# coreyjadams/SparseEventID

Hardware: NVIDIA B200
Metric: 3D sparse ResNet train events/sec (higher is better)
Workload: dtype bf16

## Files before the change

sparseeventid_b200/csrc/conv_tc.cu:

```cuda
#include <cstdlib>
#include <cstring>

#include "common.cuh"
#include "tc_ptx.cuh"

namespace tc {

constexpr int BM = 128;
constexpr int KC = 64;
constexpr int KC_TF32 = 32;
constexpr int A_BYTES = BM * 128;
constexpr int EPI_WARPS = 4;
constexpr int NGRP = 4;
constexpr int PROD_WARPS = 4 * NGRP;
constexpr int WARP_MMA = EPI_WARPS + PROD_WARPS;
constexpr int MMA_WARPS = 4;
constexpr int WARP_BLOAD = WARP_MMA + MMA_WARPS;
constexpr int THREADS = 32 * (WARP_BLOAD + 1);
constexpr int MAX_A = 12, MAX_B = 8;
constexpr int MASK_BYTES = 32;
constexpr int LIST_BYTES = 64 * 8;
using namespace tcptx;

__device__ __forceinline__ uint64_t make_desc_sw128(uint32_t saddr) {
  uint64_t d = 0;
  d |= (uint64_t)((saddr & 0x3FFFFu) >> 4);
  d |= (uint64_t)1 << 16;
  d |= (uint64_t)(1024 >> 4) << 32;
  d |= (uint64_t)1 << 46;
  d |= (uint64_t)2 << 61;
  return d;
}
__device__ __forceinline__ const unsigned char* mad_wide16(uint32_t units, const unsigned char* base) {
  uint64_t r;
  asm("mad.wide.u32 %0, %1, 16, %2;" : "=l"(r) : "r"(units), "l"((uint64_t)(uintptr_t)base));
  return reinterpret_cast<const unsigned char*>((uintptr_t)r);
}
template <bool TF32>
__device__ __forceinline__ uint32_t make_idesc(int n) {
  constexpr uint32_t fmt = TF32 ? 2u : 1u;
  return (1u << 4) | (fmt << 7) | (fmt << 10) | ((uint32_t)(n >> 3) << 17) | ((uint32_t)(BM >> 4) << 24);
}
template <bool TF32>
__device__ __forceinline__ void store8(void* out, int64_t idx, const float* f) {
  if constexpr (TF32) {
    float4* d = reinterpret_cast<float4*>(reinterpret_cast<float*>(out) + idx);
    d[0] = make_float4(f[0], f[1], f[2], f[3]);
    d[1] = make_float4(f[4], f[5], f[6], f[7]);
  } else {
    uint4 u;
    u.x = pack_bf16x2(f[0], f[1]); u.y = pack_bf16x2(f[2], f[3]);
    u.z = pack_bf16x2(f[4], f[5]); u.w = pack_bf16x2(f[6], f[7]);
    *reinterpret_cast<uint4*>(reinterpret_cast<__nv_bfloat16*>(out) + idx) = u;
  }
}
struct Params {
  const void* in;
  const int32_t* nbr;
  const unsigned char* bimg;
  const float* bias;
  void* out;
  int64_t n_rows, n_pad;
  int K, n_in, n_out;
  int nch;
  int last_kc;
  int T;
  int SA, SB;
  int num_tiles;
  int NM;
  int nbuf;
  int ksplit;
  unsigned long long* dbg;
  int exp;
};

template <int NCH, bool PAIR, bool TF32 = false>
__global__ void __launch_bounds__(THREADS, 1) k_conv_tc(const Params p) {
  static_assert(!(TF32 && PAIR), "a 32-channel fp32 row fills a stage");
  constexpr int ESZ = TF32 ? 4 : 2;
  constexpr int KCE = 128 / ESZ;
  const int nch = NCH > 0 ? NCH : p.nch;
  extern __shared__ unsigned char smem_raw[];
  pdl_launch_dependents();
  const uint32_t raw = smem_u32(smem_raw);
  const uint32_t base = (raw + 1023u) & ~1023u;
  unsigned char* gbase = smem_raw + (base - raw);
  const int SA = p.SA, SB = p.SB;
  const uint32_t b_bytes = (uint32_t)p.n_out * 128u;
  const uint32_t a_base = base;
  const uint32_t b_base = base + (uint32_t)SA * A_BYTES;
  const uint32_t bar0 = b_base + (uint32_t)SB * b_bytes;
  auto afull = [&](int s) { return bar0 + 8u * (uint32_t)s; };
  auto aempty = [&](int s) { return bar0 + 8u * (uint32_t)(MAX_A + s); };
  auto bfull = [&](int s) { return bar0 + 8u * (uint32_t)(2 * MAX_A + s); };
  auto bempty = [&](int s) { return bar0 + 8u * (uint32_t)(2 * MAX_A + MAX_B + s); };
  auto accf = [&](int b) { return bar0 + 8u * (uint32_t)(2 * MAX_A + 2 * MAX_B + b); };
  auto acce = [&](int b) { return bar0 + 8u * (uint32_t)(2 * MAX_A + 2 * MAX_B + 2 + b); };
  constexpr int NBAR = 2 * MAX_A + 2 * MAX_B + 4;
  unsigned char* tail = gbase + (size_t)SA * A_BYTES + (size_t)SB * b_bytes + 8 * NBAR;
  uint32_t* tmem_slot = reinterpret_cast<uint32_t*>(tail);
  uint32_t* amask = reinterpret_cast<uint32_t*>(tail + 16);
  unsigned char* lists = tail + 16 + MAX_A * MASK_BYTES;

  const int warp = __shfl_sync(0xffffffffu, (int)(threadIdx.x >> 5), 0), lane = threadIdx.x & 31;
  auto mark = [&](int role, int stage, int ev) {
#ifdef SCN_TC_TIMELINE
    if (p.dbg != nullptr && blockIdx.x == 0 && lane == 0 && stage < 256)
      p.dbg[((size_t)role * 256 + stage) * 8 + ev] = (unsigned long long)clock64();
#else
    (void)role; (void)stage; (void)ev;
#endif
  };
#ifdef SCN_TC_TIMELINE
  const int exp_flags = p.exp;
#else
  constexpr int exp_flags = 0;
#endif

  const int T = p.T;
  const int tile_lo = (int)(((int64_t)p.num_tiles * blockIdx.x) / gridDim.x);
  const int tile_hi = (int)(((int64_t)p.num_tiles * (blockIdx.x + 1)) / gridDim.x);
  const int my_tiles = tile_hi - tile_lo;
  const int my_groups = (my_tiles + T - 1) / T;
  auto tiles_in_group = [&](int g) { return my_tiles - g * T < T ? my_tiles - g * T : T; };
  const int NSTEP = PAIR ? (p.K + 1) / 2 : p.K;
  const int Q = NSTEP * nch;
  const bool ksplit = p.ksplit != 0 && p.NM == 2 && my_tiles == 1;

  if (warp == WARP_MMA) {
    if (lane == 0) {
      for (int s = 0; s < SA; ++s) {
        mbar_init(afull(s), 132);
        mbar_init(aempty(s), 1);
      }
      for (int s = 0; s < SB; ++s) {
        mbar_init(bfull(s), 1);
        mbar_init(bempty(s), ksplit ? 1 : p.NM);
      }
      for (int b = 0; b < 2; ++b) {
        mbar_init(accf(b), p.NM);
        mbar_init(acce(b), EPI_WARPS);
      }
      asm volatile("fence.mbarrier_init.release.cluster;" ::: "memory");
    }
    __syncwarp();
    asm volatile("tcgen05.alloc.cta_group::1.sync.aligned.shared::cta.b32 [%0], %1;" ::"r"(smem_u32(tmem_slot)), "r"(512)
                 : "memory");
    asm volatile("tcgen05.relinquish_alloc_permit.cta_group::1.sync.aligned;" ::: "memory");
  }
  tc_fence_before();
  __syncthreads();
  tc_fence_after();
  const uint32_t tmem_base = *tmem_slot;
  pdl_wait();

  const int NM = p.NM;
  const int spc = SA / NM;

  if (warp >= EPI_WARPS && warp < EPI_WARPS + PROD_WARPS) {
    const int pw = warp - EPI_WARPS;
    const int grp = pw >> 2, wq = pw & 3;
    const int cls = grp % NM, sub = grp / NM, gpc = NGRP / NM;
    constexpr int LPI = PAIR ? 4 : 8;
    constexpr int IPP = 32 / LPI;
    const int chunk = lane % LPI, isub = lane / LPI;
    const uint32_t row_vec = (uint32_t)p.n_in >> (TF32 ? 2 : 3);
    const int last_chunks = p.last_kc * ESZ / 16;
    const uint32_t lt = (1u << lane) - 1u;
    const uint32_t csw = (uint32_t)chunk << 4;
    const uint32_t myrow = 32u * (uint32_t)wq + (uint32_t)lane;
    const uint32_t drow = a_base + (myrow << 7) + ((myrow & 7u) << 4);

    int t = cls, q = 0, cc = 0, g = 0, tv = my_groups > 0 ? tiles_in_group(0) : 0;
    const int32_t* gptr = p.nbr + (int64_t)tile_lo * BM + myrow;
    const int32_t* qptr = gptr;
    const int64_t qstride = (int64_t)p.n_pad * (PAIR ? 2 : 1);
    auto next_q = [&]() {
      ++q;
      if (++cc == nch) { cc = 0; qptr += qstride; }
    };
    auto step = [&]() {
      if (ksplit) {
        next_q(); next_q();
        if (q >= Q) { g = my_groups; tv = 0; }
        return;
      }
      t += NM;
      if (t >= tv) {
        t = cls;
        next_q();
        if (q == Q) {
          q = 0; ++g;
          gptr += (int64_t)T * BM;
          qptr = gptr;
          tv = g < my_groups ? tiles_in_group(g) : 0;
        }
      }
    };
    auto valid = [&]() { return g < my_groups && (ksplit ? q < Q : cls < tv); };
    if (ksplit) {
      t = 0;
      if (cls == 1) next_q();
    }
    for (int i = 0; i < sub; ++i)
      if (valid()) step();
    auto fetch = [&](int& jl_, int& jh_, int& q_) {
      q_ = -1; jl_ = -1; jh_ = -1;
      if (valid()) {
        const int32_t* src = qptr + t * BM;
        jl_ = ldg_nc32(src);
        if (PAIR && (2 * q + 1 < p.K)) jh_ = ldg_nc32(src + p.n_pad);
        q_ = (q << 3) | cc;
        for (int i = 0; i < gpc; ++i) step();
      }
    };

    int ls = sub;
    uint32_t round = 0;
    int it = 0;
    auto do_stage = [&](const int jl, const int jh, const int qc) {
      if (wq == 0) mark(grp, it, 0);
      int2* list = reinterpret_cast<int2*>(lists + (pw * 2 + (it & 1)) * LIST_BYTES);
      const int slot = cls * spc + ls;
      const int ccur = qc & 7;
      const bool full = qc < (ksplit ? 16 : 8);
      const uint32_t dst = drow + (uint32_t)slot * A_BYTES;
      const uint32_t bl = __ballot_sync(0xffffffffu, jl >= 0);
      const uint32_t bh = PAIR ? __ballot_sync(0xffffffffu, jh >= 0) : 0u;
      int nlive;
      if (full) {
        list[lane] = make_int2(jl >= 0 ? (int)((uint32_t)jl * row_vec) : -1, (int)dst);
        if (PAIR) list[32 + lane] = make_int2(jh >= 0 ? (int)((uint32_t)jh * row_vec) : -1, (int)(dst ^ 0x40u));
        nlive = PAIR ? 64 : 32;
      } else {
        const int2 el = make_int2((int)((uint32_t)jl * row_vec), (int)dst);
        const int2 eh = make_int2((int)((uint32_t)jh * row_vec), (int)(dst ^ 0x40u));
        if (jl >= 0) list[__popc(bl & lt)] = el;
        nlive = __popc(bl);
        if (PAIR) {
          if (jh >= 0) list[nlive + __popc(bh & lt)] = eh;
          nlive += __popc(bh);
        }
        if (nlive & (IPP - 1)) {
          const bool from_hi = PAIR && bh != 0u;
          const int top = 31 - __clz(from_hi ? bh : bl);
          const int lx = __shfl_sync(0xffffffffu, from_hi ? eh.x : el.x, top);
          const int ly = __shfl_sync(0xffffffffu, from_hi ? eh.y : el.y, top);
          const int padded = (nlive + IPP - 1) & ~(IPP - 1);
          if (nlive + lane < padded) list[nlive + lane] = make_int2(lx, ly);
        }
      }
      __syncwarp();
      if (wq == 0) mark(grp, it, 1);

      mbar_wait(aempty(slot), (round & 1u) ^ 1u);
      if (wq == 0) mark(grp, it, 2);
      if (lane == 0) {
        amask[slot * 8 + wq] = ~bl;
        if (PAIR) amask[slot * 8 + 4 + wq] = ~bh;
      }
      const int npass = (nlive + IPP - 1) / IPP;
      const bool lane_on = PAIR ? true : chunk < (ccur == nch - 1 ? last_chunks : 8);
      const unsigned char* src0 = reinterpret_cast<const unsigned char*>(p.in) + ((uint32_t)ccur * 128u + csw);
      if (lane_on && !(exp_flags & 1)) {
        if (!full) {
          for (int p0 = 0; p0 < npass; p0 += 4) {
            int2 e[4];
#pragma unroll
            for (int u = 0; u < 4; ++u)
              if (p0 + u < npass) e[u] = list[(p0 + u) * IPP + isub];
#pragma unroll
            for (int u = 0; u < 4; ++u)
              if (p0 + u < npass) cp_async16((uint32_t)e[u].y ^ csw, mad_wide16((uint32_t)e[u].x, src0), 16u);
          }
        } else {
#pragma unroll
          for (int pass = 0; pass < 8; ++pass) {
            const int2 e = list[pass * IPP + isub];
            const bool live = e.x != -1;
            cp_async16((uint32_t)e.y ^ csw, mad_wide16(live ? (uint32_t)e.x : 0u, src0), live ? 16u : 0u);
          }
        }
      }
      cp_async_arrive_noinc(afull(slot));
      if (lane == 0) mbar_arrive(afull(slot));
      if (wq == 0) mark(grp, it, 3);
      ++it;
      ls += gpc;
      if (ls >= spc) { ls -= spc; ++round; }
    };

    int jlA, jhA, qA, jlB, jhB, qB;
    fetch(jlA, jhA, qA);
    fetch(jlB, jhB, qB);
    while (qA >= 0) {
      int jlC, jhC, qC;
      fetch(jlC, jhC, qC);
      do_stage(jlA, jhA, qA);
      jlA = jlB; jhA = jhB; qA = qB;
      jlB = jlC; jhB = jhC; qB = qC;
    }
  } else if (warp == WARP_BLOAD) {
    const int total_b = my_groups * Q;
    int bslot = 0;
    uint32_t bround = 0;
    for (int i = 0; i < total_b; ++i) {
      mark(8, i, 0);
      if (ksplit) mbar_wait_sleep(bempty(bslot), (bround & 1u) ^ 1u, 100u);
      else mbar_wait(bempty(bslot), (bround & 1u) ^ 1u);
      mark(8, i, 1);
      if (elect_one()) {
        mbar_expect_tx(bfull(bslot), b_bytes);
        bulk_g2s(b_base + (uint32_t)bslot * b_bytes, p.bimg + (size_t)(i % Q) * b_bytes, b_bytes, bfull(bslot));
      }
      __syncwarp();
      if (++bslot == SB) { bslot = 0; ++bround; }
    }
  } else if (warp >= WARP_MMA && warp < WARP_MMA + MMA_WARPS) {
    const int m = warp - WARP_MMA;
    if (m < NM) {
      const uint32_t idesc = make_idesc<TF32>(p.n_out);
      const uint64_t da0 = make_desc_sw128(a_base), db0 = make_desc_sw128(b_base);
      const int nbuf = p.nbuf;
      int bslot = 0;
      uint32_t bround = 0;
      int ls = 0;
      uint32_t around = 0;
      int it = 0;
      auto issue_stage = [&](int q, uint32_t col, uint64_t db, bool first) {
        const int cc = PAIR ? 0 : q % nch;
        const int step = PAIR ? q : q / nch;
        const int nk = PAIR ? ((2 * step + 1 < p.K) ? 4 : 2) : ((cc == nch - 1 ? p.last_kc : KCE) * ESZ / 32);
        const int aslot = m * spc + ls;
        mark(4 + m, it, 0);
        mbar_wait(afull(aslot), around & 1u);
        mark(4 + m, it, 1);
        tc_fence_after();
        uint32_t m0 = 0, m1 = 0, m2 = 0, m3 = 0, h0 = 0, h1 = 0, h2 = 0, h3 = 0;
        if (!first) {
          const uint4 mw = *reinterpret_cast<const uint4*>(amask + aslot * 8);
          m0 = __ballot_sync(0xffffffffu, (mw.x >> lane) & 1u);
          m1 = __ballot_sync(0xffffffffu, (mw.y >> lane) & 1u);
          m2 = __ballot_sync(0xffffffffu, (mw.z >> lane) & 1u);
          m3 = __ballot_sync(0xffffffffu, (mw.w >> lane) & 1u);
          if (PAIR) {
            const uint4 hw = *reinterpret_cast<const uint4*>(amask + aslot * 8 + 4);
            h0 = __ballot_sync(0xffffffffu, (hw.x >> lane) & 1u);
            h1 = __ballot_sync(0xffffffffu, (hw.y >> lane) & 1u);
            h2 = __ballot_sync(0xffffffffu, (hw.z >> lane) & 1u);
            h3 = __ballot_sync(0xffffffffu, (hw.w >> lane) & 1u);
          }
        }
        const uint64_t da = da0 + (uint64_t)((uint32_t)aslot * (A_BYTES >> 4));
        const uint32_t tmem_d = tmem_base + col;
        if (elect_one()) {
#pragma unroll
          for (int kk = 0; kk < 4; ++kk) {
            if (kk < nk && !(exp_flags & 2)) {
              const bool hi = PAIR && kk >= 2;
              umma_masked<TF32>(tmem_d, da + (uint64_t)(kk * 2), db + (uint64_t)(kk * 2), idesc, (!first || kk > 0) ? 1u : 0u,
                                hi ? h0 : m0, hi ? h1 : m1, hi ? h2 : m2, hi ? h3 : m3);
            }
          }
          umma_commit(aempty(aslot));
        }
        __syncwarp();
        mark(4 + m, it, 2);
        ++it;
        if (++ls == spc) { ls = 0; ++around; }
      };
      if (ksplit) {
        mbar_wait(acce(0), 1u);
        tc_fence_after();
        bslot = m;
        for (int q = m; q < Q; q += 2) {
          mbar_wait(bfull(bslot), bround & 1u);
          issue_stage(q, (uint32_t)(m * p.n_out), db0 + (uint64_t)(((uint32_t)bslot * b_bytes) >> 4), q < 2);
          if (elect_one()) umma_commit(bempty(bslot));
          __syncwarp();
          bslot += 2;
          if (bslot >= SB) { bslot -= SB; ++bround; }
        }
        if (elect_one()) umma_commit(accf(0));
        __syncwarp();
      } else
      for (int g = 0; g < my_groups; ++g) {
        const int buf = nbuf == 2 ? (g & 1) : 0;
        const uint32_t use = (uint32_t)(nbuf == 2 ? (g >> 1) : g);
        const int tv = tiles_in_group(g);
        mbar_wait(acce(buf), (use & 1u) ^ 1u);
        tc_fence_after();
        for (int q = 0; q < Q; ++q) {
          mark(10 + m, g * Q + q, 0);
          mbar_wait(bfull(bslot), bround & 1u);
          mark(10 + m, g * Q + q, 1);
          const uint64_t db = db0 + (uint64_t)(((uint32_t)bslot * b_bytes) >> 4);
          for (int t = m; t < tv; t += NM) issue_stage(q, (uint32_t)buf * 256u + (uint32_t)(t * p.n_out), db, q == 0);
          if (elect_one()) umma_commit(bempty(bslot));
          __syncwarp();
          if (++bslot == SB) { bslot = 0; ++bround; }
        }
        if (elect_one()) umma_commit(accf(buf));
        __syncwarp();
      }
    }
  } else if (warp < EPI_WARPS) {
    if (ksplit) {
      mbar_wait_sleep(accf(0), 0u, 100u);
      tc_fence_after();
      const int64_t row = (int64_t)tile_lo * BM + warp * 32 + lane;
      const uint32_t taddr = tmem_base + ((uint32_t)(warp * 32) << 16);
      for (int c0 = 0; c0 < p.n_out; c0 += 16) {
        uint32_t a[16], b[16];
        tmem_ld16x2(taddr + (uint32_t)c0, taddr + (uint32_t)(p.n_out + c0), a, b);
        if (row < p.n_rows && !(exp_flags & 4)) {
#pragma unroll
          for (int gq = 0; gq < 2; ++gq) {
            float f[8];
#pragma unroll
            for (int e = 0; e < 8; ++e)
              f[e] = __uint_as_float(a[gq * 8 + e]) + __uint_as_float(b[gq * 8 + e]) +
                     (p.bias ? __ldg(p.bias + c0 + gq * 8 + e) : 0.f);
            store8<TF32>(p.out, row * p.n_out + c0 + gq * 8, f);
          }
        }
      }
      tc_fence_before();
    } else
    for (int g = 0; g < my_groups; ++g) {
      const int buf = p.nbuf == 2 ? (g & 1) : 0;
      if (warp == 0) mark(9, g, 0);
      mbar_wait_long(accf(buf), (uint32_t)(p.nbuf == 2 ? (g >> 1) : g) & 1u);
      if (warp == 0) mark(9, g, 1);
      tc_fence_after();
      const int tv = tiles_in_group(g);
      for (int t = 0; t < tv; ++t) {
        const int64_t tile = (int64_t)tile_lo + (int64_t)g * T + t;
        const int64_t row = tile * BM + warp * 32 + lane;
        const uint32_t taddr = tmem_base + ((uint32_t)(warp * 32) << 16) + (uint32_t)buf * 256u + (uint32_t)(t * p.n_out);
        for (int c0 = 0; c0 < p.n_out; c0 += 32) {
          uint32_t v[32];
          tmem_ld32(taddr + (uint32_t)c0, v);
          if (row < p.n_rows && !(exp_flags & 4)) {
#pragma unroll
            for (int gq = 0; gq < 4; ++gq) {
              float f[8];
#pragma unroll
              for (int e = 0; e < 8; ++e)
                f[e] = __uint_as_float(v[gq * 8 + e]) + (p.bias ? __ldg(p.bias + c0 + gq * 8 + e) : 0.f);
              store8<TF32>(p.out, row * p.n_out + c0 + gq * 8, f);
            }
          }
        }
      }
      tc_fence_before();
      __syncwarp();
      if (warp == 0) mark(9, g, 2);
      if (lane == 0) mbar_arrive(acce(buf));
    }
  }

  tc_fence_before();
  __syncthreads();
  if (warp == WARP_MMA) {
    tc_fence_after();
    asm volatile("tcgen05.dealloc.cta_group::1.sync.aligned.b32 %0, %1;" ::"r"(tmem_base), "r"(512) : "memory");
  }
}

__global__ void k_prep_weights_tc(const float* __restrict__ W, int K, int Cin, int Cout, int transpose, int mirror,
                                  int nch, int pair, int tf32, void* __restrict__ img) {
  const int n_in = transpose ? Cout : Cin, n_out = transpose ? Cin : Cout;
  int64_t total = (int64_t)K * n_in * n_out;
  int64_t i = blockIdx.x * (int64_t)blockDim.x + threadIdx.x;
  if (i >= total) return;
  int k = (int)(i / ((int64_t)n_in * n_out));
  int rem = (int)(i - (int64_t)k * n_in * n_out);
  int n = rem / n_in, c = rem % n_in;
  int src_k = (transpose && mirror) ? K - 1 - k : k;
  int ci = transpose ? n : c, co = transpose ? c : n;
  float v = W[((int64_t)src_k * Cin + ci) * Cout + co];
  if (tf32) {
    const int q = k * nch + c / KC_TF32, chunk = (c % KC_TF32) >> 2;
    reinterpret_cast<float*>(img)[((size_t)q * n_out + n) * 32 + (size_t)((chunk ^ (n & 7)) << 2) + (c & 3)] = to_tf32_rna(v);
    return;
  }
  const int q = pair ? (k >> 1) : k * nch + c / KC;
  const int chunk = pair ? (k & 1) * 4 + (c >> 3) : (c % KC) >> 3;
  size_t off = ((size_t)q * n_out + n) * 64 + (size_t)((chunk ^ (n & 7)) << 3) + (c & 7);
  reinterpret_cast<__nv_bfloat16*>(img)[off] = __float2bfloat16_rn(v);
}

__global__ void __launch_bounds__(256) k_prep_weights_tc_batched(const long long* __restrict__ descs, int n, long long units) {
  pdl_launch_dependents();
  pdl_wait();
  const long long i = blockIdx.x * (long long)blockDim.x + threadIdx.x;
  if (i >= units) return;
  const long long e = i * 8;
  int lo = 0, hi = n - 1;
  while (lo < hi) {
    const int mid = (lo + hi + 1) >> 1;
    if (__ldg(descs + mid * 8 + 6) <= e) lo = mid; else hi = mid - 1;
  }
  const long long* d = descs + lo * 8;
  const float* W = reinterpret_cast<const float*>(d[0]);
  unsigned char* img = reinterpret_cast<unsigned char*>(d[1]);
  const int K = (int)d[2], Cin = (int)d[3], Cout = (int)d[4], transpose = (int)(d[5] & 1), mirror = (int)((d[5] >> 1) & 1);
  const int n_in = transpose ? Cout : Cin, n_out = transpose ? Cin : Cout;
  const bool tf32 = d[7] == SCN_PREC_TF32;
  const int kc = tf32 ? KC_TF32 : KC;
  const int nch = (n_in + kc - 1) / kc, pair = !tf32 && n_in == 32;
  const int u = (int)((e - d[6]) >> 3);
  const int per_k = (n_in >> 3) * n_out;
  const int k = u / per_k;
  const int r = u - k * per_k;
  const int cb = r / n_out, nn = r - cb * n_out;
  const int c0 = cb * 8;
  const int src_k = (transpose && mirror) ? K - 1 - k : k;
  float v[8];
  if (transpose) {
    const float4* src = reinterpret_cast<const float4*>(W + ((long long)src_k * Cin + nn) * Cout + c0);
    const float4 a = __ldg(src), b = __ldg(src + 1);
    v[0] = a.x; v[1] = a.y; v[2] = a.z; v[3] = a.w; v[4] = b.x; v[5] = b.y; v[6] = b.z; v[7] = b.w;
  } else {
    const float* src = W + ((long long)src_k * Cin + c0) * Cout + nn;
#pragma unroll
    for (int j = 0; j < 8; ++j) v[j] = __ldg(src + (long long)j * Cout);
  }
  if (tf32) {
    const int q = k * nch + c0 / KC_TF32, chunk = (c0 % KC_TF32) >> 2;
    unsigned char* row = img + ((size_t)q * n_out + nn) * 128;
    *reinterpret_cast<float4*>(row + ((chunk ^ (nn & 7)) << 4)) =
        make_float4(to_tf32_rna(v[0]), to_tf32_rna(v[1]), to_tf32_rna(v[2]), to_tf32_rna(v[3]));
    *reinterpret_cast<float4*>(row + (((chunk + 1) ^ (nn & 7)) << 4)) =
        make_float4(to_tf32_rna(v[4]), to_tf32_rna(v[5]), to_tf32_rna(v[6]), to_tf32_rna(v[7]));
    return;
  }
  const int q = pair ? (k >> 1) : k * nch + c0 / KC;
  const int chunk = pair ? (k & 1) * 4 + cb : (c0 % KC) >> 3;
  uint4 o;
  o.x = pack_bf16x2(v[0], v[1]); o.y = pack_bf16x2(v[2], v[3]);
  o.z = pack_bf16x2(v[4], v[5]); o.w = pack_bf16x2(v[6], v[7]);
  *reinterpret_cast<uint4*>(img + ((size_t)q * n_out + nn) * 128 + (size_t)((chunk ^ (nn & 7)) << 4)) = o;
}

}

extern "C" int scn_conv_prep_weights_batched(const void* descs, int n, int64_t total, void* stream) {
  if (n <= 0 || total <= 0) return SCN_OK;
  if (!descs) return SCN_ERR_ARG;
  SCN_CUDA(scn_launch_pdl(tc::k_prep_weights_tc_batched, dim3(grid_for(total / 8, 256)), dim3(256), 0, (cudaStream_t)stream,
                          (const long long*)descs, n, (long long)(total / 8)));
  SCN_LAUNCH_CHECK();
  return SCN_OK;
}

static unsigned long long* g_tc_dbg = nullptr;
extern "C" void scn_tc_debug_timeline(void* device_buffer) { g_tc_dbg = (unsigned long long*)device_buffer; }
#ifdef SCN_TC_TIMELINE
static int g_tc_exp = 0;
extern "C" void scn_tc_debug_exp(int flags) { g_tc_exp = flags; }
#else
extern "C" void scn_tc_debug_exp(int) {}
#endif

bool scn_tc_shape_ok(int K, int n_in, int n_out) {
  return K >= 1 && (n_in % 32) == 0 && (n_out % 32) == 0 && n_in >= 32 && n_in <= 256 && n_out >= 32 && n_out <= 256;
}

static bool tc_pair(int n_in, int tf32) { return !tf32 && n_in == 32; }
static int tc_nch(int n_in, int tf32) {
  const int kc = tf32 ? tc::KC_TF32 : tc::KC;
  return (n_in + kc - 1) / kc;
}

size_t scn_tc_image_bytes(int K, int n_in, int n_out, int tf32) {
  const size_t stages = tc_pair(n_in, tf32) ? (size_t)(K + 1) / 2 : (size_t)K * tc_nch(n_in, tf32);
  return stages * n_out * 128;
}

int scn_tc_prep(const float* W, int K, int Cin, int Cout, int transpose, int mirror, int tf32, void* out, cudaStream_t s) {
  const int n_in = transpose ? Cout : Cin, n_out = transpose ? Cin : Cout;
  const int nch = tc_nch(n_in, tf32);
  if (!tf32 && (n_in % tc::KC) != 0) SCN_CUDA(cudaMemsetAsync(out, 0, scn_tc_image_bytes(K, n_in, n_out, tf32), s));
  int64_t total = (int64_t)K * Cin * Cout;
  tc::k_prep_weights_tc<<<grid_for(total, 256), 256, 0, s>>>(W, K, Cin, Cout, transpose, mirror, nch,
                                                             tc_pair(n_in, tf32) ? 1 : 0, tf32, out);
  SCN_LAUNCH_CHECK();
  return SCN_OK;
}

static int env_int(const char* name) {
  const char* e = std::getenv(name);
  return e ? std::atoi(e) : 0;
}
static int g_knob[4] = {-1, -1, -1, -1};
extern "C" void scn_tc_debug_knobs(int grid, int t, int sa, int sb) {
  g_knob[0] = grid; g_knob[1] = t; g_knob[2] = sa; g_knob[3] = sb;
}
static int32_t g_last_launch[9] = {0, 0, 0, 0, 0, 0, 0, 0, 0};
extern "C" void scn_tc_debug_last_launch(int32_t* out) {
  for (int i = 0; i < 9; ++i) out[i] = g_last_launch[i];
}

int scn_tc_forward(const void* in, int64_t n_in_rows, const int32_t* nbr, int K, int64_t n_rows, int64_t n_pad, int n_in,
                   int n_out, const void* bimg, const float* bias, void* out, int tf32, cudaStream_t s) {
  const uint64_t row_units = (uint64_t)n_in * (tf32 ? 4u : 2u) / 16u;
  if ((uint64_t)n_in_rows * row_units >= 0xffffffffull) return SCN_ERR_UNSUPPORTED;
  if (g_knob[0] < 0) {
    g_knob[0] = env_int("SCN_B200_TC_GRID"); g_knob[1] = env_int("SCN_B200_TC_T");
    g_knob[2] = env_int("SCN_B200_TC_SA"); g_knob[3] = env_int("SCN_B200_TC_SB");
  }
  const int force_grid = g_knob[0], force_t = g_knob[1], force_sa = g_knob[2], force_sb = g_knob[3];
  tc::Params p;
  p.dbg = g_tc_dbg;
#ifdef SCN_TC_TIMELINE
  p.exp = g_tc_exp;
#else
  p.exp = 0;
#endif
  p.in = in; p.nbr = nbr; p.bimg = (const unsigned char*)bimg; p.bias = bias; p.out = out;
  p.n_rows = n_rows; p.n_pad = n_pad; p.K = K; p.n_in = n_in; p.n_out = n_out;
  const bool pair = tc_pair(n_in, tf32);
  const int nch = tc_nch(n_in, tf32);
  p.nch = nch;
  p.last_kc = n_in - (nch - 1) * (tf32 ? tc::KC_TF32 : tc::KC);
  p.num_tiles = (int)((n_rows + tc::BM - 1) / tc::BM);
  int max_ctas = kNumSMs;
  if (force_grid > 0 && force_grid < max_ctas) max_ctas = force_grid;
  const int per_cta = (p.num_tiles + max_ctas - 1) / max_ctas;
  const int q_per_tile = (pair ? (K + 1) / 2 : K) * nch;
  int T = 1;
  p.nbuf = 2;
  {
    double best = 1e30;
    for (int t = 1; t <= 8 && t * n_out <= 512 && t <= (per_cta > 0 ? per_cta : 1); ++t) {
      const int nm = t >= 4 ? 4 : (t >= 2 ? 2 : 1);
      const int full = per_cta / t, rem = per_cta % t;
      const int groups = full + (rem ? 1 : 0);
      const double units = (double)full * ((t + nm - 1) / nm) + (rem ? (rem + nm - 1) / nm : 0);
      const int nbuf = t * n_out <= 256 ? 2 : 1;
      const double ep = (double)t * (n_out / 32.0) * 600.0 / ((double)q_per_tile * 1400.0);
      const double cost = units + (nbuf == 1 ? groups * ep : ep + 0.15 * (groups - 1) * ep);
      if (cost <= best + 1e-9) { best = cost; T = t; p.nbuf = nbuf; }
    }
  }
  if (force_t > 0) {
    T = force_t;
    if (T > 8) T = 8;
    if (T * n_out > 512) T = 512 / n_out;
    if (T > per_cta) T = per_cta;
    if (T < 1) T = 1;
    p.nbuf = T * n_out <= 256 ? 2 : 1;
  }
  p.T = T;
  p.NM = T >= 4 ? 4 : (T >= 2 ? 2 : 1);
  p.ksplit = 0;
  const int stages_per_tile = (pair ? (K + 1) / 2 : K) * nch;
  if (stages_per_tile >= 2) {
    if (p.NM == 1 && per_cta == 1 && 2 * n_out <= 512) { p.NM = 2; p.nbuf = 1; p.ksplit = 1; }
    else if (p.NM == 2) p.ksplit = 1;
  }
  const uint32_t b_bytes = (uint32_t)n_out * 128u;
  constexpr int NBAR = 2 * tc::MAX_A + 2 * tc::MAX_B + 4;
  const uint32_t fixed = 1024u + 8u * NBAR + 16u + (uint32_t)tc::MAX_A * tc::MASK_BYTES +
                         2u * (uint32_t)tc::PROD_WARPS * tc::LIST_BYTES + 16u;
  const uint32_t budget = 226u * 1024u - fixed;
  int SA = 8;
  if (p.ksplit && per_cta <= 2) SA = 4;
  if (force_sa > 0) SA = force_sa;
  SA = SA / tc::NGRP * tc::NGRP;
  if (SA > tc::MAX_A) SA = tc::MAX_A;
  if (SA < tc::NGRP) SA = tc::NGRP;
  while (SA > tc::NGRP && (uint32_t)SA * tc::A_BYTES + 2u * b_bytes > budget) SA -= tc::NGRP;
  if ((uint32_t)SA * tc::A_BYTES + 2u * b_bytes > budget) return SCN_ERR_UNSUPPORTED;
  int SB = (int)((budget - (uint32_t)SA * tc::A_BYTES) / b_bytes);
  if (SB > tc::MAX_B) SB = tc::MAX_B;
  if (force_sb >= 2 && force_sb < SB) SB = force_sb;
  if (p.ksplit && (SB & 1)) --SB;
  p.SA = SA;
  p.SB = SB;
  const size_t smem = (size_t)fixed + (size_t)SA * tc::A_BYTES + (size_t)SB * b_bytes;
  int grid = p.num_tiles < max_ctas ? p.num_tiles : max_ctas;
  {
    static bool attr_set = false;
    if (!attr_set) {
      SCN_CUDA(cudaFuncSetAttribute(tc::k_conv_tc<1, true>, cudaFuncAttributeMaxDynamicSharedMemorySize, 227 * 1024));
      SCN_CUDA(cudaFuncSetAttribute(tc::k_conv_tc<1, false>, cudaFuncAttributeMaxDynamicSharedMemorySize, 227 * 1024));
      SCN_CUDA(cudaFuncSetAttribute(tc::k_conv_tc<2, false>, cudaFuncAttributeMaxDynamicSharedMemorySize, 227 * 1024));
      SCN_CUDA(cudaFuncSetAttribute(tc::k_conv_tc<3, false>, cudaFuncAttributeMaxDynamicSharedMemorySize, 227 * 1024));
      SCN_CUDA(cudaFuncSetAttribute(tc::k_conv_tc<4, false>, cudaFuncAttributeMaxDynamicSharedMemorySize, 227 * 1024));
      SCN_CUDA(cudaFuncSetAttribute(tc::k_conv_tc<0, false, true>, cudaFuncAttributeMaxDynamicSharedMemorySize, 227 * 1024));
      attr_set = true;
    }
  }
  if (grid < 1) return SCN_OK;
  {
    const int32_t rec[9] = {grid, p.T, p.NM, p.nbuf, p.ksplit, p.SA, p.SB, p.num_tiles / grid,
                            (p.num_tiles + grid - 1) / grid};
    for (int i = 0; i < 9; ++i) g_last_launch[i] = rec[i];
  }
  auto launch = [&](auto kern) -> int {
    SCN_CUDA(scn_launch_pdl(kern, dim3((unsigned)grid), dim3(tc::THREADS), smem, s, p));
    SCN_LAUNCH_CHECK();
    return SCN_OK;
  };
  if (tf32) return nch <= 8 ? launch(tc::k_conv_tc<0, false, true>) : SCN_ERR_UNSUPPORTED;
  if (pair) return launch(tc::k_conv_tc<1, true>);
  switch (nch) {
    case 1: return launch(tc::k_conv_tc<1, false>);
    case 2: return launch(tc::k_conv_tc<2, false>);
    case 3: return launch(tc::k_conv_tc<3, false>);
    case 4: return launch(tc::k_conv_tc<4, false>);
    default: return SCN_ERR_UNSUPPORTED;
  }
}
```

Before: 3563.

## Split K-steps across MMA warps for underfilled last tile group

When a CTA's final tile group has at most half as many tiles as MMA warps, each tile's K-steps are split between two MMA warps that accumulate into separate TMEM regions. The epilogue then sums the two partial accumulators. This generalizes the existing single-tile ksplit path so idle MMA warps help on the tail group, and the T-selection cost model is updated to value such tails at half a unit. It adds extra TMEM usage and extra epilogue loads in exchange for better tensor-core utilization on the tail.

```diff
diff --git a/sparseeventid_b200/csrc/conv_tc.cu b/sparseeventid_b200/csrc/conv_tc.cu
--- a/sparseeventid_b200/csrc/conv_tc.cu
+++ b/sparseeventid_b200/csrc/conv_tc.cu
@@ -126,6 +126,10 @@
   const int NSTEP = PAIR ? (p.K + 1) / 2 : p.K;
   const int Q = NSTEP * nch;
   const bool ksplit = p.ksplit != 0 && p.NM == 2 && my_tiles == 1;
+  const int tv_last = my_groups > 0 ? tiles_in_group(my_groups - 1) : 0;
+  const bool split_last = !ksplit && T >= p.NM && my_groups > 0 && 2 * tv_last <= p.NM && Q >= 2 &&
+                          2 * tv_last * p.n_out <= (p.nbuf == 2 ? 256 : 512);
+  auto is_split = [&](int g) { return split_last && g == my_groups - 1; };
 
   if (warp == WARP_MMA) {
     if (lane == 0) {
@@ -179,8 +183,12 @@
       ++q;
       if (++cc == nch) { cc = 0; qptr += qstride; }
     };
+    auto enter_split = [&]() {
+      t = cls >> 1;
+      if (cls & 1) next_q();
+    };
     auto step = [&]() {
-      if (ksplit) {
+      if (ksplit || is_split(g)) {
         next_q(); next_q();
         if (q >= Q) { g = my_groups; tv = 0; }
         return;
@@ -194,13 +202,18 @@
           gptr += (int64_t)T * BM;
           qptr = gptr;
           tv = g < my_groups ? tiles_in_group(g) : 0;
+          if (is_split(g)) enter_split();
         }
       }
     };
-    auto valid = [&]() { return g < my_groups && (ksplit ? q < Q : cls < tv); };
+    auto valid = [&]() {
+      return g < my_groups && (ksplit ? q < Q : is_split(g) ? (cls < 2 * tv && q < Q) : cls < tv);
+    };
     if (ksplit) {
       t = 0;
       if (cls == 1) next_q();
+    } else if (is_split(0)) {
+      enter_split();
     }
     for (int i = 0; i < sub; ++i)
       if (valid()) step();
@@ -210,7 +223,7 @@
         const int32_t* src = qptr + t * BM;
         jl_ = ldg_nc32(src);
         if (PAIR && (2 * q + 1 < p.K)) jh_ = ldg_nc32(src + p.n_pad);
-        q_ = (q << 3) | cc;
+        q_ = ((ksplit || is_split(g)) ? q < 2 : q == 0) ? 8 | cc : cc;
         for (int i = 0; i < gpc; ++i) step();
       }
     };
@@ -223,7 +236,7 @@
       int2* list = reinterpret_cast<int2*>(lists + (pw * 2 + (it & 1)) * LIST_BYTES);
       const int slot = cls * spc + ls;
       const int ccur = qc & 7;
-      const bool full = qc < (ksplit ? 16 : 8);
+      const bool full = (qc & 8) != 0;
       const uint32_t dst = drow + (uint32_t)slot * A_BYTES;
       const uint32_t bl = __ballot_sync(0xffffffffu, jl >= 0);
       const uint32_t bh = PAIR ? __ballot_sync(0xffffffffu, jh >= 0) : 0u;
@@ -395,7 +408,11 @@
           mbar_wait(bfull(bslot), bround & 1u);
           mark(10 + m, g * Q + q, 1);
           const uint64_t db = db0 + (uint64_t)(((uint32_t)bslot * b_bytes) >> 4);
-          for (int t = m; t < tv; t += NM) issue_stage(q, (uint32_t)buf * 256u + (uint32_t)(t * p.n_out), db, q == 0);
+          if (!is_split(g)) {
+            for (int t = m; t < tv; t += NM) issue_stage(q, (uint32_t)buf * 256u + (uint32_t)(t * p.n_out), db, q == 0);
+          } else if (m < 2 * tv && (q & 1) == (m & 1)) {
+            issue_stage(q, (uint32_t)buf * 256u + (uint32_t)(m * p.n_out), db, q < 2);
+          }
           if (elect_one()) umma_commit(bempty(bslot));
           __syncwarp();
           if (++bslot == SB) { bslot = 0; ++bround; }
@@ -405,11 +422,7 @@
       }
     }
   } else if (warp < EPI_WARPS) {
-    if (ksplit) {
-      mbar_wait_sleep(accf(0), 0u, 100u);
-      tc_fence_after();
-      const int64_t row = (int64_t)tile_lo * BM + warp * 32 + lane;
-      const uint32_t taddr = tmem_base + ((uint32_t)(warp * 32) << 16);
+    auto store_pair = [&](int64_t row, uint32_t taddr) {
       for (int c0 = 0; c0 < p.n_out; c0 += 16) {
         uint32_t a[16], b[16];
         tmem_ld16x2(taddr + (uint32_t)c0, taddr + (uint32_t)(p.n_out + c0), a, b);
@@ -425,6 +438,11 @@
           }
         }
       }
+    };
+    if (ksplit) {
+      mbar_wait_sleep(accf(0), 0u, 100u);
+      tc_fence_after();
+      store_pair((int64_t)tile_lo * BM + warp * 32 + lane, tmem_base + ((uint32_t)(warp * 32) << 16));
       tc_fence_before();
     } else
     for (int g = 0; g < my_groups; ++g) {
@@ -437,7 +455,12 @@
       for (int t = 0; t < tv; ++t) {
         const int64_t tile = (int64_t)tile_lo + (int64_t)g * T + t;
         const int64_t row = tile * BM + warp * 32 + lane;
-        const uint32_t taddr = tmem_base + ((uint32_t)(warp * 32) << 16) + (uint32_t)buf * 256u + (uint32_t)(t * p.n_out);
+        const uint32_t tbase = tmem_base + ((uint32_t)(warp * 32) << 16) + (uint32_t)buf * 256u;
+        if (is_split(g)) {
+          store_pair(row, tbase + (uint32_t)(2 * t * p.n_out));
+          continue;
+        }
+        const uint32_t taddr = tbase + (uint32_t)(t * p.n_out);
         for (int c0 = 0; c0 < p.n_out; c0 += 32) {
           uint32_t v[32];
           tmem_ld32(taddr + (uint32_t)c0, v);
@@ -638,7 +661,8 @@
       const int nm = t >= 4 ? 4 : (t >= 2 ? 2 : 1);
       const int full = per_cta / t, rem = per_cta % t;
       const int groups = full + (rem ? 1 : 0);
-      const double units = (double)full * ((t + nm - 1) / nm) + (rem ? (rem + nm - 1) / nm : 0);
+      const double last = rem == 0 ? 0.0 : (2 * rem <= nm && q_per_tile >= 2) ? 0.5 : (double)((rem + nm - 1) / nm);
+      const double units = (double)full * ((t + nm - 1) / nm) + last;
       const int nbuf = t * n_out <= 256 ? 2 : 1;
       const double ep = (double)t * (n_out / 32.0) * 600.0 / ((double)q_per_tile * 1400.0);
       const double cost = units + (nbuf == 1 ? groups * ep : ep + 0.15 * (groups - 1) * ep);
```

Result: faster. 3625, median of 6 (+1.8%).
